# Rouslan/NTracer

Measured on AMD Instinct MI355X. Metric: Mrays/s (primary+shadow), 6-D hypercube @1920x1080, higher is better.
Workload: dtype f32

## Files before the change

ntracer_amd/csrc/nt_box.hpp:

```cpp
#pragma once
#include <type_traits>
#include "nt_pixel.hpp"

namespace {

__device__ __forceinline__ bool box_may_hit(int n, const float *dots, float sx, float sy, float sq) {
    const float osq = dots[0];
    const float ov = fmaf(-dots[2], sy, fmaf(dots[1], sx, dots[3]));
    const float rad2 = (float)n * (1.0f + NT_FUZZ) * (1.0f + NT_FUZZ) * 1.001f;
#ifdef NT_EXP_SKIP_SLABS
    return false;
#else
    return !((osq - rad2) * sq > ov * ov * 1.0001f);
#endif
}

__device__ __forceinline__ void box_background(float in, float &r, float &g, float &b) {
    if (in > 0.0f) { r = in; g = in; b = in; }
    else { r = 0.0f; g = -in; b = -in; }
}

template <int N>
__device__ __forceinline__ void box_color(const float (&o)[N], const float (&dir)[N], bool maybe, float &r, float &g, float &b) {
    bool done = false;
    float shade = 0.0f;

    {
        float num[N];
        bool pre[N];
        float aK = 0.0f, bK = 1.0f, oK = 0.0f;
        bool any = false;
#pragma unroll
        for (int i = 0; i < N; ++i) {
            const float di = dir[i];
            const float s = di < 0.0f ? 1.0f : -1.0f;
            num[i] = s - o[i];
            pre[i] = maybe && ((num[i] > 0.0f && di > 0.0f) || (num[i] < 0.0f && di < 0.0f));
            const float a = fabsf(num[i]), bb = fabsf(di);
            if (pre[i] && (!any || a * bK > aK * bb)) { aK = a; bK = bb; oK = o[i]; any = true; }
        }
        const float mu = 1e-4f * (1.0f + fabsf(oK));
        const float aKm = (aK - mu) * (1.0f - 1e-6f);
#pragma unroll
        for (int i = 0; i < N; ++i) {
            const bool tie = pre[i] && !done && !(fabsf(num[i]) * bK < fabsf(dir[i]) * aKm);
            if (__builtin_amdgcn_ballot_w64(tie) != 0ull) {
                const float di = dir[i];
                const float dist = num[i] / di;
                bool ok = tie && dist > 0.0f;
#pragma unroll
                for (int j = 0; j < N; ++j) {
                    if (j != i) {
                        const float p = dir[j] * dist + o[j];
                        ok = ok && !(fabsf(p) > (1.0f + NT_FUZZ));
                    }
                }
                if (ok) {
                    done = true;
                    if (dist >= FLT_MAX) shade = -1.0f;
                    else {
                        const float sine = di * (di < 0.0f ? 1.0f : -1.0f);
                        shade = sine <= 0.0f ? -sine : 0.0f;
                    }
                }
            }
        }
    }
    if (done && shade >= 0.0f) {
        r = shade * 1.0f;
        g = shade * 0.5f;
        b = shade * 0.5f;
    } else {
        box_background(dir[0], r, g, b);
    }
}

#ifndef NT_BOX_INLINE_MAX_N
#define NT_BOX_INLINE_MAX_N 8
#endif
#ifndef NT_BOX_SETS_MAX_N
#define NT_BOX_SETS_MAX_N NT_BOX_INLINE_MAX_N
#endif
#ifndef NT_BOX_MARGIN
#define NT_BOX_MARGIN 1e-5f
#endif
template <int N>
__device__ __forceinline__ void box_classify(const float (&o)[N], const float (&v)[N], float m, bool maybe, bool &hit, bool &unclear,
                                             float &x, float (&near)[N], float &tn, float &vK) {
    float tn2 = -INFINITY;
    tn = -INFINITY;
    vK = 0.0f;
    float tnp = -INFINITY, tfp = INFINITY;
    const float m1p = 1.0f + m;
#pragma unroll
    for (int j = 0; j < N; ++j) {
        const float inv = __builtin_amdgcn_rcpf(v[j]);
        const float c0 = -o[j] * inv;
        const float nr = c0 - fabsf(inv);
        near[j] = nr;
        tnp = fmaxf(tnp, fmaf(-fabsf(inv), m1p, c0));
        tfp = fminf(tfp, fmaf(fabsf(inv), m1p, c0));
        const bool later = nr > tn;
        tn2 = __builtin_amdgcn_fmed3f(tn, tn2, nr);
        vK = later ? v[j] : vK;
        tn = fmaxf(tn, nr);
    }
    const bool miss = tnp > tfp || tfp < 0.0f;
    const float c = 1.0f - m;
    float sum = 0.0f;
#pragma unroll
    for (int j = 0; j < N; ++j) sum = sum + fmaxf(fabsf(fmaf(v[j], tn, o[j])), c);
    const bool inside = sum - (float)N * c <= 1.5f * m;
    const bool sole = (tn - tn2) * fabsf(vK) > m;
    const bool front = tn > 1e-3f && tn < 1e30f;
    hit = maybe && !miss && inside && sole && front;
    unclear = maybe && !miss && !hit;
#ifdef NT_EXP_NOUNCLEAR
    unclear = false;
#endif
    x = hit ? vK : v[0];
}

__device__ __forceinline__ float nt_vmax(float a, float b) { float r; asm("v_max_f32 %0, %1, %2" : "=v"(r) : "v"(a), "v"(b)); return r; }
__device__ __forceinline__ float nt_vmin(float a, float b) { float r; asm("v_min_f32 %0, %1, %2" : "=v"(r) : "v"(a), "v"(b)); return r; }
__device__ __forceinline__ float nt_vmax3(float a, float b, float c) { float r; asm("v_max3_f32 %0, %1, %2, %3" : "=v"(r) : "v"(a), "v"(b), "v"(c)); return r; }
__device__ __forceinline__ float nt_vmin3(float a, float b, float c) { float r; asm("v_min3_f32 %0, %1, %2, %3" : "=v"(r) : "v"(a), "v"(b), "v"(c)); return r; }
__device__ __forceinline__ float nt_vmed3(float a, float b, float c) { float r; asm("v_med3_f32 %0, %1, %2, %3" : "=v"(r) : "v"(a), "v"(b), "v"(c)); return r; }
__device__ __forceinline__ float nt_vmax_abs(float a, float b) { float r; asm("v_max_f32 %0, |%1|, %2" : "=v"(r) : "v"(a), "v"(b)); return r; }

#ifndef NT_BOX_CLASSIFY_SETS_MIN_N
#define NT_BOX_CLASSIFY_SETS_MIN_N 6
#endif
#ifndef NT_BOX_CLASSIFY_SETS_MAX_N
#define NT_BOX_CLASSIFY_SETS_MAX_N 7
#endif
template <int N>
__device__ __forceinline__ void box_classify_sets(const float (&o)[N], const float (&v)[N], float m, uint32_t sets, bool &hit, bool &unclear,
                                                  float &x) {
    float tn = -INFINITY, tn2 = -INFINITY, vK = 0.0f;
    float tnp = -INFINITY, tfp = INFINITY;
    const float m1p = 1.0f + m;
#pragma unroll
    for (int j = 0; j < N; ++j) {
        if (((sets >> (10 + j)) & 1u) != 0u) {
            const float inv = __builtin_amdgcn_rcpf(v[j]);
            const float c0 = -o[j] * inv;
            tfp = nt_vmin(tfp, fmaf(fabsf(inv), m1p, c0));
            if (((sets >> j) & 1u) != 0u) {
                const float nr = c0 - fabsf(inv);
                tnp = nt_vmax(tnp, fmaf(-fabsf(inv), m1p, c0));
                const bool later = nr > tn;
                tn2 = nt_vmed3(tn, tn2, nr);
                vK = later ? v[j] : vK;
                tn = nt_vmax(tn, nr);
            }
        }
    }
    const bool miss = tnp > tfp || tfp < 0.0f;
    const float c = 1.0f - m;
    float sum = 0.0f;
#pragma unroll
    for (int j = 0; j < N; ++j) {
        if (((sets >> (10 + j)) & 1u) != 0u) {
            asm volatile("" : "+v"(sum));
            sum = sum + nt_vmax_abs(fmaf(v[j], tn, o[j]), c);
        }
    }
    const bool inside = sum - (float)__builtin_popcount((sets >> 10) & 0x3ffu) * c <= 1.5f * m;
    const bool sole = (tn - tn2) * fabsf(vK) > m;
    const bool front = tn > 1e-3f && tn < 1e30f;
    hit = !miss && inside && sole && front;
    unclear = !miss && !hit;
    x = hit ? vK : v[0];
}

template <int N>
__device__ __forceinline__ void box_entries(const float (&o)[N], const float (&v)[N], float (&near)[N], float &tn, float &vK) {
    tn = -INFINITY;
    vK = 0.0f;
#pragma unroll
    for (int j = 0; j < N; ++j) {
        const float inv = __builtin_amdgcn_rcpf(v[j]);
        const float nr = fmaf(-o[j], inv, -fabsf(inv));
        near[j] = nr;
        vK = nr > tn ? v[j] : vK;
        tn = fmaxf(tn, nr);
    }
}

template <int N>
__device__ __forceinline__ void box_resolve(const float (&o)[N], const float (&v)[N], float len, float m, const float (&near)[N], float tn,
                                            float vK, bool unclear, bool &hit, float &x) {
    const float aK = fabsf(vK);
    const float slack = m * __builtin_amdgcn_rcpf(aK), lim = 1.0f - 0.5f * m;
    bool inT[N], inC[N];
    float d[N];
    uint32_t anyC = 0u;
#pragma unroll
    for (int j = 0; j < N; ++j) {
        const bool early = (tn - near[j]) * aK > m;
        const bool robust = fmaf(fabsf(v[j]), slack, fabsf(fmaf(v[j], tn, o[j]))) <= lim;
        inT[j] = unclear && !early;
        inC[j] = unclear && !(robust && early);
        d[j] = 0.0f;
        if (__builtin_amdgcn_ballot_w64(inC[j]) != 0ull) {
            d[j] = v[j] / len;
            anyC |= 1u << j;
        }
    }
    bool done = false, found = false;
    float xs = v[0];
#pragma unroll
    for (int i = 0; i < N; ++i) {
        const bool cand = inT[i] && !done;
        if (__builtin_amdgcn_ballot_w64(cand) != 0ull) {
            const float di = d[i];
            const float dist = ((di < 0.0f ? 1.0f : -1.0f) - o[i]) / di;
            bool ok = cand && di != 0.0f && dist > 0.0f;
#pragma unroll
            for (int j = 0; j < N; ++j) {
                if (j != i && ((anyC >> j) & 1u) != 0u) {
                    const float p = d[j] * dist + o[j];
                    ok = ok && !(inC[j] && fabsf(p) > (1.0f + NT_FUZZ));
                }
            }
            if (ok) {
                done = true;
                if (!(dist >= FLT_MAX)) { found = true; xs = v[i]; }
            }
        }
    }
    if (unclear) {
        hit = found;
        x = xs;
    }
}

typedef __attribute__((address_space(1))) uint8_t *nt_gptr;
__device__ __forceinline__ nt_gptr uniform_ptr(uint8_t *p) {
    const unsigned long long v = reinterpret_cast<unsigned long long>(p);
    const uint32_t lo = (uint32_t)__builtin_amdgcn_readfirstlane((int)(uint32_t)v), hi = (uint32_t)__builtin_amdgcn_readfirstlane((int)(uint32_t)(v >> 32));
    return (nt_gptr)(((unsigned long long)hi << 32) | lo);
}
#define NT_G32(p) (*(__attribute__((address_space(1))) uint32_t *)(p))

template <typename P>
__device__ __forceinline__ void emit_f32x3_at(const NtTarget &tg, P p, float r, float gb) {
    r = r > 0.0f ? r : 0.0f;
    r = r < 1.0f ? r : 1.0f;
    gb = gb > 0.0f ? gb : 0.0f;
    gb = gb < 1.0f ? gb : 1.0f;
    uint32_t vr = __float_as_uint(r), vgb = __float_as_uint(gb);
    uint3 w;
    if (tg.plain_f32[0] == 0 && tg.plain_f32[1] == 1 && tg.plain_f32[2] == 2 && !tg.reversed) {
        w.x = bswap32(vr);
        w.y = bswap32(vgb);
        w.z = w.y;
    } else {
        if (!tg.reversed) { vr = bswap32(vr); vgb = bswap32(vgb); }
        w.x = tg.plain_f32[tg.reversed ? 2 : 0] == 0 ? vr : vgb;
        w.y = tg.plain_f32[1] == 0 ? vr : vgb;
        w.z = tg.plain_f32[tg.reversed ? 0 : 2] == 0 ? vr : vgb;
    }
    if constexpr (std::is_same<P, nt_gptr>::value) {
        typedef uint32_t u32x3 __attribute__((ext_vector_type(3)));
        u32x3 v;
        v.x = w.x; v.y = w.y; v.z = w.z;
        *(__attribute__((address_space(1))) u32x3 *)(p) = v;
    } else {
        *reinterpret_cast<uint3 *>(p) = w;
    }
}
__device__ __forceinline__ void emit_f32x3(const NtTarget &tg, long long offset, float r, float gb) { emit_f32x3_at(tg, tg.dest + offset, r, gb); }

__device__ __forceinline__ float sqrt_in_range(float x) {
    const float s = __builtin_amdgcn_sqrtf(x);
    const float s_dn = __uint_as_float(__float_as_uint(s) - 1u), s_up = __uint_as_float(__float_as_uint(s) + 1u);
    const float vp = fmaf(-s_dn, s, x), vs = fmaf(-s_up, s, x);
    float r = vp <= 0.0f ? s_dn : s;
    r = vs > 0.0f ? s_up : r;
    return r;
}
__device__ __forceinline__ float sqrt_wave(float x) {
    if (__builtin_amdgcn_ballot_w64(!(x >= 0x1p-96f && x < 0x1p96f)) == 0ull) return sqrt_in_range(x);
    return sqrtf(x);
}

template <int N, bool PLAIN, bool DEFER = false, bool REDO = false, bool F32 = false>
__device__ __forceinline__ bool box_pixel(const NtTarget &tg, const PixelRef &pr, const float (&org)[N], float (&dir)[N], float sq,
                                          const float (&dots)[4], float sx, float sy, float margin, bool rowhit = true, int face = -1,
                                          uint32_t sets = 0u, bool noclass = false) {
    constexpr bool INL = (F32 || PLAIN) && !REDO && !DEFER;
    const bool redo = REDO || (INL && noclass);
    const bool maybe = redo || (rowhit && (DEFER || INL || box_may_hit(N, dots, sx, sy, sq)));
    float r, g, b;
    bool hit = false, unclear = false;
    float x = dir[0];
#ifndef NT_EXP_NOCLASSIFY
    float near[N], tn = 0.0f, vK = 0.0f;
    constexpr bool CSETS = INL && N >= NT_BOX_CLASSIFY_SETS_MIN_N && N <= NT_BOX_CLASSIFY_SETS_MAX_N;
    auto exact_on_sets = [&]() {
        const float len = sqrt_wave(sq);
        float d[N];
#pragma unroll
        for (int j = 0; j < N; ++j) {
            d[j] = 0.0f;
            if ((sets >> (10 + j)) & 1u) d[j] = dir[j] / len;
        }
        bool done = false;
        x = dir[0];
#pragma unroll
        for (int i = 0; i < N; ++i) {
            if (((sets >> i) & 1u) != 0u && __builtin_amdgcn_ballot_w64(!done) != 0ull) {
// ... 245 lines not shown
    }
}

template <int N, bool SETS = false>
__device__ __forceinline__ unsigned long long box_stretch_code2(const float (&org)[N], const float (&right)[N], const float (&up)[N],
                                                                const float (&fwd)[N], const NtTarget &tg, int y, int col) {
    uint32_t sets_value = 0u;
    uint32_t *const sets = SETS ? &sets_value : nullptr;
    uint32_t code = 0u;
    float omax = fabsf(org[0]);
#pragma unroll
    for (int j = 1; j < N; ++j) omax = fmaxf(omax, fabsf(org[j]));
    const float m = NT_BOX_MARGIN * (1.0f + omax);
    const float h = 1.0f + 2.0f * m + 1e-3f;
    const float sxc = tg.fovI * (((float)(col * 64) + 31.5f) - tg.half_w);
    const float sy = tg.fovI * ((float)y - tg.half_h);
    const float spread = 32.0f * tg.fovI;
    float tlo = 0.0f, thi = INFINITY;
    float vc[N], g[N];
    float tn = -INFINITY, tn2 = -INFINITY, vK = 0.0f, gK = 0.0f, oK = 0.0f;
    int K = 0;
#pragma unroll
    for (int j = 0; j < N; ++j) {
        vc[j] = (fwd[j] + right[j] * sxc) - up[j] * sy;
        g[j] = fmaf(spread, fabsf(right[j]), 1e-6f);
        const float pa = vc[j] + g[j], qa = -h - org[j];
        const float pb = vc[j] - g[j], qb = h - org[j];
        const float ra = qa * __builtin_amdgcn_rcpf(pa), rb = qb * __builtin_amdgcn_rcpf(pb);
        const bool ap = pa >= 0.0f, bp = pb >= 0.0f;
        const float lo_a = ap ? ra : -INFINITY, hi_a = ap ? INFINITY : ra;
        const float hi_b = bp ? rb : INFINITY, lo_b = bp ? -INFINITY : rb;
        tlo = nt_vmax3(tlo, lo_a, lo_b);
        thi = nt_vmin3(thi, hi_a, hi_b);
    }
    if (!(tlo > thi)) {
        code = 15u;
#pragma unroll
        for (int j = 0; j < N; ++j) {
            const float nr = ((vc[j] < 0.0f ? 1.0f : -1.0f) - org[j]) * __builtin_amdgcn_rcpf(vc[j]);
            tn2 = nt_vmed3(tn, tn2, nr);
            const bool later = nr > tn;
            vK = later ? vc[j] : vK;
            gK = later ? g[j] : gK;
            oK = later ? org[j] : oK;
            K = later ? j : K;
            tn = nt_vmax(tn, nr);
        }
        const float vKa = vK - gK, vKb = vK + gK;
        if (K < 13 && vKa * vKb > 0.0f) {
            const float num = (vK < 0.0f ? 1.0f : -1.0f) - oK;
            const float t1 = num * __builtin_amdgcn_rcpf(vKa), t2 = num * __builtin_amdgcn_rcpf(vKb);
            const float t_lo = nt_vmin(t1, t2) * (1.0f - 1e-6f), t_hi = nt_vmax(t1, t2) * (1.0f + 1e-6f);
            const float rK = m * __builtin_amdgcn_rcpf(fabsf(vK) - gK) * (1.0f + 1e-6f);
            bool ok = t_lo > 1e-3f && t_hi < 1e30f;
#pragma unroll
            for (int j = 0; j < N; ++j) {
                const float va = vc[j] - g[j], vb = vc[j] + g[j];
                const float pmax = org[j] + nt_vmax(vb * t_lo, vb * t_hi);
                const float pmin = org[j] + nt_vmin(va * t_lo, va * t_hi);
                const float lim = (1.0f - m - 1e-4f) - (fabsf(vc[j]) + g[j]) * rK;
                ok = ok && (j == K || (pmax <= lim && pmin >= -lim));
            }
            if (ok) code = (uint32_t)K + 1u;
        }
        if (code == 15u && !((tn - tn2) * fabsf(vK) > m)) code = 14u;
        if (code >= 14u) {
            if (sets != nullptr && N <= 10) {
                auto range = [&](int j, float &A, float &B, float &vabs) {
                    const float va = vc[j] - g[j], vb = vc[j] + g[j];
                    const float num = (vc[j] < 0.0f ? 1.0f : -1.0f) - org[j];
                    const float e1 = num * __builtin_amdgcn_rcpf(va), e2 = num * __builtin_amdgcn_rcpf(vb);
                    const float lo = nt_vmin(e1, e2), hi = nt_vmax(e1, e2);
                    const bool same = va * vb > 0.0f;
                    A = same ? lo - fabsf(lo) * 1e-6f : -INFINITY;
                    B = same ? hi + fabsf(hi) * 1e-6f : INFINITY;
                    vabs = same ? fabsf(vc[j]) - g[j] : 0.0f;
                };
                float rA[N], rB[N], rV[N];
                float TN = -INFINITY, TH = -INFINITY;
#pragma unroll
                for (int j = 0; j < N; ++j) {
                    range(j, rA[j], rB[j], rV[j]);
                    TN = nt_vmax(TN, rA[j]);
                    TH = nt_vmax(TH, rB[j]);
                }
                float vmin = INFINITY;
#pragma unroll
                for (int j = 0; j < N; ++j) vmin = rB[j] >= TN ? nt_vmin(vmin, rV[j]) : vmin;
                const float M = m * __builtin_amdgcn_rcpf(vmin) * (1.0f + 1e-5f);
                uint32_t T = 0u, C = 0u;
                float t_lo = INFINITY;
                const float t_hi = TH;
#pragma unroll
                for (int j = 0; j < N; ++j) {
                    const bool inT = rB[j] >= TN - M;
                    T |= inT ? 1u << j : 0u;
                    t_lo = inT ? nt_vmin(t_lo, rA[j]) : t_lo;
                }
#pragma unroll
                for (int j = 0; j < N; ++j) {
                    const float va = vc[j] - g[j], vb = vc[j] + g[j];
                    const float pmax = org[j] + nt_vmax(vb * t_lo, vb * t_hi);
                    const float pmin = org[j] + nt_vmin(va * t_lo, va * t_hi);
                    const float lim = 1.0f - m - 1e-4f;
                    const bool inC = ((T >> j) & 1u) != 0u || !(pmax <= lim && pmin >= -lim);
                    C |= inC ? 1u << j : 0u;
                }
                const bool valid = vmin > 0.0f && t_lo > 1e-3f && t_hi < 1e30f;
                *sets = valid ? (0x80000000u | (C << 10) | T) : 0u;
            }
        }
    }
    return (unsigned long long)code | ((unsigned long long)sets_value << 32);
}
template <int N>
__device__ __forceinline__ uint32_t box_stretch_code(const float (&org)[N], const float (&right)[N], const float (&up)[N], const float (&fwd)[N],
                                                     const NtTarget &tg, int y, int col) {
    return (uint32_t)box_stretch_code2<N, false>(org, right, up, fwd, tg, y, col);
}

template <int N>
__global__ __launch_bounds__(256) void box_cull_kernel(NtCameraFixed cam, NtTarget tg, uint32_t *out, int ncols) {
    float org[N], right[N], up[N], fwd[N];
    load_camera<N>(cam, org, right, up, fwd);
    const int word = (int)blockIdx.x, row = (int)blockIdx.y * 8 + (int)(threadIdx.x >> 5);
    const int col = word * 32 + (int)(threadIdx.x & 31);
    uint32_t code = 0u;
    if (row < tg.row_count && col < ncols) {
        const int orow = tg.row_begin + row;
        int y = orow;
        if (tg.band_world > 1) {
            const int band = orow / tg.band_rows;
            y = (band * tg.band_world + tg.band_rank) * tg.band_rows + (orow - band * tg.band_rows);
        }
        code = box_stretch_code<N>(org, right, up, fwd, tg, y, col);
    }
    uint32_t packed = code << (4 * (threadIdx.x & 7));
    packed |= (uint32_t)__shfl_xor((int)packed, 1, 64);
    packed |= (uint32_t)__shfl_xor((int)packed, 2, 64);
    packed |= (uint32_t)__shfl_xor((int)packed, 4, 64);
    if (row < tg.row_count && (threadIdx.x & 7) == 0) out[((size_t)blockIdx.z * tg.row_count + row) * tg.cull_words + (col >> 3)] = packed;
}

#ifdef NT_EXP_NOSTORE
#define NT_EXP_STORE_IF if (tg.width < 0)
#else
#define NT_EXP_STORE_IF
#endif
#ifndef NT_TILE_OCC
#define NT_TILE_OCC
#endif
#ifndef NT_BOX_PIN_UP
#define NT_BOX_PIN_UP 1
#endif
template <int N, bool F32, int ROWS, int WAVES>
__global__ __launch_bounds__(64 * WAVES) NT_TILE_OCC void box_tile_kernel(NtCameraFixed cam, NtTarget tg) {
    static_assert(ROWS == 8 || ROWS == 16 || ROWS == 32 || ROWS == 64, "sixteen row codes to a qword, one to four qwords a wave");
    static_assert(WAVES >= 1 && WAVES <= 4 && WAVES * ROWS <= 64, "the codes of a tile are the work of one wave, a row per lane");
    constexpr int R = ROWS;
    __shared__ uint32_t s_code[64];
    __shared__ unsigned long long s_rows[4];
    constexpr bool ALLIN = F32 || N <= NT_BOX_INLINE_MAX_N;
    constexpr bool SETS_LDS = ALLIN && N <= NT_BOX_SETS_MAX_N;
    __shared__ uint32_t s_sets[SETS_LDS ? 64 : 1];
    __shared__ int s_abort;
    const int tid = (int)threadIdx.x;
    const int lane = tid & 63;
    const int wv = __builtin_amdgcn_readfirstlane(tid >> 6);
#ifdef NT_EXP_TRACE
    const unsigned long long trace_t0 = wall_clock64();
    unsigned trace_rows = 0u;
    unsigned long long trace_t1 = 0ull;
#endif
    const unsigned nframes = gridDim.z - (unsigned)tg.lead_frames;
    unsigned frame = blockIdx.z;
    if (tg.lead_frames > 0) {
        const unsigned cols = gridDim.x, q = cols / 4u;
        const bool middle = blockIdx.x >= q && blockIdx.x < cols - q;
        if (!middle) frame -= (unsigned)tg.lead_frames;
        if (frame >= nframes) return;
    }
    float org[N], right[N], up[N], fwd[N], dir[N];
    load_camera<N>(cam, frame, org, right, up, fwd);
    float margin = fabsf(org[0]);
#pragma unroll
    for (int j = 1; j < N; ++j) margin = fmaxf(margin, fabsf(org[j]));
    margin = NT_BOX_MARGIN * (1.0f + margin);
    float dots[4];
    if (cam.buf) {
        const float *dp = cam.dots + (size_t)frame * 4;
        dots[0] = dp[0]; dots[1] = dp[1]; dots[2] = dp[2]; dots[3] = dp[3];
    } else {
        dots[0] = cam.odots[0]; dots[1] = cam.odots[1]; dots[2] = cam.odots[2]; dots[3] = cam.odots[3];
    }
    const int tile_row0 = (int)blockIdx.y * WAVES * R;
    if (wv == (int)((blockIdx.x + blockIdx.y + frame) % (unsigned)WAVES)) {
        if (tg.abort_word != nullptr) {
            const bool ab = nt_aborted(tg);
            if (WAVES == 1) { if (ab) return; }
            else if (lane == 0) s_abort = ab ? 1 : 0;
        }
        uint32_t code = 0u;
        uint32_t row_sets = 0u;
        const int trow = tg.row_il > 0 ? ((int)blockIdx.y * WAVES + lane / R) + tg.row_il * (lane % R) : tile_row0 + lane;
        if (lane < WAVES * R && trow < tg.row_count) {
            const int orow = tg.row_begin + trow;
            int y = orow;
            if (tg.band_world > 1) {
                const int band = orow / tg.band_rows;
                y = (band * tg.band_world + tg.band_rank) * tg.band_rows + (orow - band * tg.band_rows);
            }
            if (y < tg.height) {
                const unsigned long long cs = box_stretch_code2<N, (N <= NT_BOX_SETS_MAX_N)>(org, right, up, fwd, tg, y, (int)blockIdx.x);
                code = (uint32_t)cs;
                row_sets = (uint32_t)(cs >> 32);
            }
        }
        if (SETS_LDS) s_sets[lane] = row_sets;
        {
            const unsigned long long m0 = __builtin_amdgcn_ballot_w64(code == 0u), m1 = __builtin_amdgcn_ballot_w64(code >= 1u && code <= 13u),
                                     m2 = __builtin_amdgcn_ballot_w64(code == 15u), m3 = __builtin_amdgcn_ballot_w64(code == 14u);
            if (lane == 0) {
                s_rows[0] = m0;
                s_rows[1] = m1;
                s_rows[2] = m2;
                s_rows[3] = m3;
            }
        }
        uint32_t packed = code << (4 * (lane & 7));
        packed |= (uint32_t)__shfl_xor((int)packed, 1, 64);
        packed |= (uint32_t)__shfl_xor((int)packed, 2, 64);
        packed |= (uint32_t)__shfl_xor((int)packed, 4, 64);
        if ((lane & 7) == 0) {
            const int grp = lane >> 3;
            const int slot = R == 8 ? 2 * grp : grp;
            s_code[slot] = packed;
            if (R == 8) s_code[slot + 1] = 0u;
        }
    }
    __syncthreads();
    if (WAVES > 1 && tg.abort_word != nullptr && s_abort != 0) return;
#ifdef NT_EXP_TRACE
    trace_t1 = wall_clock64();
#endif
    constexpr int HALVES = R >= 32 ? R / 16 : 1, RH = R / HALVES;
    const int wrow0 = tile_row0 + wv * R;
    const int il = tg.row_il;
    const int wfirst = il > 0 ? (int)blockIdx.y * WAVES + wv : wrow0;
    if (wfirst < tg.row_count) {
        typedef uint32_t nt_u32x4 __attribute__((ext_vector_type(4)));
        typedef __attribute__((address_space(4))) const nt_u32x4 *nt_rowtab;
        uint8_t *const frame_base = tg.dest + (long long)frame * tg.frame_stride;
#define NT_ROW_LOAD(rr)                     \
        const nt_u32x4 row_e = tab[(rr)];   \
        const float sy = __uint_as_float(row_e.x)
#define NT_ROW_OFF() ((long long)(((unsigned long long)row_e.w << 32) | row_e.z) + (long long)frame * tg.frame_stride)
#define NT_ROW_PTR() uniform_ptr(frame_base + (long long)(((unsigned long long)row_e.w << 32) | row_e.z))
#define NT_LANE_OFF() ({ asm volatile("" : "+v"(xoff)); xoff; })
#define NT_CLEAR_BIT(mask, bit) asm("s_bitset0_b32 %0, %1" : "+s"(mask) : "s"(bit))
        int x = (int)blockIdx.x * 64 + lane;
        x = x < tg.width ? x : tg.width - 1;
        uint32_t xoff = (uint32_t)x * (uint32_t)tg.bpp;
        const float sx = tg.fovI * ((float)x - tg.half_w);
        float base[N];
#pragma unroll
        for (int j = 0; j < N; ++j) base[j] = fwd[j] + right[j] * sx;
        float upv[N];
#pragma unroll
        for (int j = 0; j < N; ++j) {
            upv[j] = up[j];
            if (NT_BOX_PIN_UP || F32 || j == 0) asm volatile("" : "+v"(upv[j]));
        }
        float bb = 0.0f, bu = 0.0f, uu = 0.0f;
        bool fastsq = true;
        if (!F32) {
#pragma unroll
            for (int j = 0; j < N; ++j) {
                bb = fmaf(base[j], base[j], bb);
                bu = fmaf(base[j], up[j], bu);
                uu = fmaf(up[j], up[j], uu);
            }
            fastsq = __builtin_amdgcn_ballot_w64(!(bu * bu <= bb * uu * 0.0625f)) == 0ull;
        }
        const float maxv = (float)tg.plain_maxval;
        const float inv_maxv2 = 1.0f / (maxv * maxv);
        const float m2bu = (-2.0f * bu) * inv_maxv2;
        bb = bb * inv_maxv2;
        uu = uu * inv_maxv2;
        auto rows_of = [&](int k) {
            const unsigned long long m = s_rows[k];
            return (((unsigned long long)(uint32_t)__builtin_amdgcn_readfirstlane((int)(uint32_t)(m >> 32)) << 32) |
                    (uint32_t)__builtin_amdgcn_readfirstlane((int)(uint32_t)m)) >> (wv * R);
        };
        const unsigned long long rows_culled = rows_of(0), rows_face = rows_of(1), rows_rays = rows_of(2), rows_tie = rows_of(3);
#pragma unroll 1
        for (int half = 0; half < HALVES; ++half) {
        const int row0 = wrow0 + 16 * half;
        const int hfirst = il > 0 ? wfirst + il * 16 * half : row0;
        if (hfirst >= tg.row_count) break;
        uint32_t redo_bits = 0u;
        const int cw = (R >= 32 ? (R / 8) * wv + 2 * half : 2 * wv);
        unsigned long long rowcodes = ((unsigned long long)(uint32_t)__builtin_amdgcn_readfirstlane((int)s_code[cw + 1]) << 32) |
                                      (uint32_t)__builtin_amdgcn_readfirstlane((int)s_code[cw]);
        const int lrow = il > 0 ? hfirst + il * lane : row0 + lane;
        const int lorow = tg.row_begin + lrow;
        int ly = lorow;
        if (tg.band_world > 1) {
            const int band = lorow / tg.band_rows;
            ly = (band * tg.band_world + tg.band_rank) * tg.band_rows + (lorow - band * tg.band_rows);
        }
        const uint32_t valid = (uint32_t)__builtin_amdgcn_ballot_w64(lane < RH && lrow < tg.row_count && ly < tg.height);
        const nt_rowtab tab = (nt_rowtab)tg.rowtab + (il > 0 ? row0 : tg.row_begin + row0);
        uint32_t quick = (uint32_t)(rows_culled >> (16 * half)) & valid, inner = (uint32_t)(rows_face >> (16 * half)) & valid;
        uint32_t todo = (uint32_t)((ALLIN ? rows_rays | rows_tie : rows_rays) >> (16 * half)) & valid;
        if (!ALLIN) redo_bits = (uint32_t)(rows_tie >> (16 * half)) & valid;
#ifdef NT_EXP_TRACE
        trace_rows += (unsigned)__builtin_popcount(quick) | ((unsigned)__builtin_popcount(inner) << 8) |
                      ((unsigned)__builtin_popcount((uint32_t)(rows_rays >> (16 * half)) & valid) << 16) |
                      ((unsigned)__builtin_popcount((uint32_t)(rows_tie >> (16 * half)) & valid) << 24);
#endif
        if (!F32) {
            if (!fastsq) {
                todo |= quick | inner;
                quick = 0u;
                inner = 0u;
            }
            auto lean_rows = [&](auto sel8) {
            constexpr bool SEL8 = decltype(sel8)::value;
            while (quick != 0u) {
                const int rr = __builtin_ctz(quick);
                NT_CLEAR_BIT(quick, rr);
                NT_ROW_LOAD(rr);
                const float d0 = base[0] - upv[0] * sy;
                const float sqa = fmaf(sy, fmaf(sy, uu, m2bu), bb);
                const float t = fabsf(d0) * __builtin_amdgcn_rsqf(sqa);
                const bool clear = fabsf(__builtin_amdgcn_fractf(t) - 0.5f) > fmaf(t, 0x1p-18f, 0x1p-18f);
                if (__builtin_amdgcn_ballot_w64(!clear) != 0ull) {
                    todo |= 1u << rr;
                    continue;
                }
                const nt_gptr out = NT_ROW_PTR() + NT_LANE_OFF();
                if (SEL8) {
                    const uint32_t q = __float_as_uint(t + 8388608.0f);
                    const uint32_t w = __builtin_amdgcn_perm(d0 > 0.0f ? q : 0u, q, tg.plain_sel);
                    NT_EXP_STORE_IF NT_G32(out) = w;
                    continue;
                }
                uint32_t q = (uint32_t)(t + 0.5f);
                q = q < tg.plain_maxval ? q : tg.plain_maxval;
                const uint32_t w = (d0 > 0.0f ? q : 0u) * tg.plain_mul[0] + q * (tg.plain_mul[1] + tg.plain_mul[2]);
                NT_EXP_STORE_IF NT_G32(out) = tg.reversed ? w : bswap32(w);
            }
            uint32_t K0 = 0u;
            float bK0 = base[0], uK0 = upv[0];
            if (inner != 0u) {
                K0 = ((uint32_t)(rowcodes >> (4 * __builtin_ctz(inner))) & 15u) - 1u;
#pragma unroll
                for (int j = 1; j < N; ++j) {
                    bK0 = K0 == (uint32_t)j ? base[j] : bK0;
                    uK0 = K0 == (uint32_t)j ? upv[j] : uK0;
                }
            }
            while (inner != 0u) {
                const int rr = __builtin_ctz(inner);
                NT_CLEAR_BIT(inner, rr);
                const uint32_t K = ((uint32_t)(rowcodes >> (4 * rr)) & 15u) - 1u;
                NT_ROW_LOAD(rr);
                float bK = bK0, uK = uK0;
                if (K != K0) {
                    bK = base[0];
                    uK = upv[0];
#pragma unroll
                    for (int j = 1; j < N; ++j) {
                        bK = K == (uint32_t)j ? base[j] : bK;
                        uK = K == (uint32_t)j ? upv[j] : uK;
                    }
                }
                const float dK = bK - uK * sy;
                const float sqa = fmaf(sy, fmaf(sy, uu, m2bu), bb);
                const float t = fabsf(dK) * __builtin_amdgcn_rsqf(sqa), th = t * 0.5f;
                const bool clear = fabsf(__builtin_amdgcn_fractf(t) - 0.5f) > fmaf(t, 0x1p-18f, 0x1p-18f) &&
                                   fabsf(__builtin_amdgcn_fractf(th) - 0.5f) > fmaf(th, 0x1p-18f, 0x1p-18f);
                if (__builtin_amdgcn_ballot_w64(!clear) != 0ull) {
                    todo |= 1u << rr;
                    continue;
                }
                const nt_gptr out = NT_ROW_PTR() + NT_LANE_OFF();
                if (SEL8) {
                    NT_EXP_STORE_IF NT_G32(out) = __builtin_amdgcn_perm(__float_as_uint(t + 8388608.0f), __float_as_uint(th + 8388608.0f), tg.plain_sel);
                    continue;
                }
                uint32_t qr = (uint32_t)(t + 0.5f), qgb = (uint32_t)(th + 0.5f);
                qr = qr < tg.plain_maxval ? qr : tg.plain_maxval;
                qgb = qgb < tg.plain_maxval ? qgb : tg.plain_maxval;
                const uint32_t w = qr * tg.plain_mul[0] + qgb * (tg.plain_mul[1] + tg.plain_mul[2]);
                NT_EXP_STORE_IF NT_G32(out) = tg.reversed ? w : bswap32(w);
            }
            };
            if (tg.plain_sel != 0u) lean_rows(std::true_type{});
            else lean_rows(std::false_type{});
        } else {
            while (quick != 0u) {
                const int rr = __builtin_ctz(quick);
                quick &= quick - 1u;
                NT_ROW_LOAD(rr);
#pragma unroll
                for (int j = 0; j < N; ++j) dir[j] = base[j] - upv[j] * sy;
                float sq = dir[0] * dir[0];
#pragma unroll
                for (int j = 1; j < N; ++j) sq = sq + dir[j] * dir[j];
                const float in = dir[0] / sqrt_wave(sq);
                float r, gb, b_;
                box_background(in, r, gb, b_);
                emit_f32x3_at(tg, NT_ROW_PTR() + NT_LANE_OFF(), r, gb);
            }
            uint32_t K0 = 0u;
            float bK0 = base[0], uK0 = upv[0];
            if (inner != 0u) {
                K0 = ((uint32_t)(rowcodes >> (4 * __builtin_ctz(inner))) & 15u) - 1u;
#pragma unroll
                for (int j = 1; j < N; ++j) {
                    bK0 = K0 == (uint32_t)j ? base[j] : bK0;
                    uK0 = K0 == (uint32_t)j ? upv[j] : uK0;
                }
            }
            while (inner != 0u) {
                const int rr = __builtin_ctz(inner);
                inner &= inner - 1u;
                const uint32_t K = ((uint32_t)(rowcodes >> (4 * rr)) & 15u) - 1u;
                NT_ROW_LOAD(rr);
#pragma unroll
                for (int j = 0; j < N; ++j) dir[j] = base[j] - upv[j] * sy;
                float sq = dir[0] * dir[0];
#pragma unroll
                for (int j = 1; j < N; ++j) sq = sq + dir[j] * dir[j];
                float bK = bK0, uK = uK0;
                if (K != K0) {
                    bK = base[0];
                    uK = upv[0];
#pragma unroll
                    for (int j = 1; j < N; ++j) {
                        bK = K == (uint32_t)j ? base[j] : bK;
                        uK = K == (uint32_t)j ? upv[j] : uK;
                    }
                }
                const float xk = bK - uK * sy;
                const float shade = fabsf(xk / sqrt_wave(sq));
                emit_f32x3_at(tg, NT_ROW_PTR() + NT_LANE_OFF(), shade * 1.0f, shade * 0.5f);
            }
        }
        while (todo != 0u) {
            const int rr = __builtin_ctz(todo);
            todo &= todo - 1u;
            const bool rowhit = ((uint32_t)(rowcodes >> (4 * rr)) & 15u) != 0u;
            NT_ROW_LOAD(rr);
            PixelRef pr;
            pr.x = x;
            pr.y = 0;
            pr.offset = NT_ROW_OFF() + (long long)xoff;
            pr.hit_index = 0;
            pr.valid = true;
#pragma unroll
            for (int j = 0; j < N; ++j) dir[j] = base[j] - upv[j] * sy;
            float sq = dir[0] * dir[0];
#pragma unroll
            for (int j = 1; j < N; ++j) sq = sq + dir[j] * dir[j];
            const int rcode = (int)((uint32_t)(rowcodes >> (4 * rr)) & 15u);
            if (ALLIN) {
                uint32_t sets = 0u;
                if (SETS_LDS) sets = (uint32_t)__builtin_amdgcn_readfirstlane((int)s_sets[wv * R + 16 * half + rr]);
                box_pixel<N, !F32, false, false, F32>(tg, pr, org, dir, sq, dots, sx, sy, margin, rowhit, rcode >= 1 && rcode <= 13 ? rcode - 1 : -1, sets,
                                                       rcode == 14);
            } else if (!box_pixel<N, true, true, false, false>(tg, pr, org, dir, sq, dots, sx, sy, margin, rowhit, rcode >= 1 && rcode <= 13 ? rcode - 1 : -1)) {
                redo_bits |= 1u << rr;
            }
        }
        if (!ALLIN && lane == 0) {
            while (redo_bits != 0u) {
                const int rr = __builtin_ctz(redo_bits);
                redo_bits &= redo_bits - 1u;
                const int mrow = il > 0 ? hfirst + il * rr : row0 + rr;
                atomicOr(tg.redo + ((size_t)frame * tg.row_count + mrow) * tg.redo_words + (blockIdx.x >> 5), 1u << (blockIdx.x & 31));
            }
        }
        }
    }
#ifdef NT_EXP_TRACE
    if (lane == 0) {
        unsigned long long *tr = reinterpret_cast<unsigned long long *>(tg.dest + (long long)nframes * tg.frame_stride) +
                                 ((((size_t)frame * gridDim.y + blockIdx.y) * gridDim.x + blockIdx.x) * WAVES + wv) * 4;
        tr[0] = trace_t0;
        tr[1] = wall_clock64();
        tr[2] = (unsigned long long)__builtin_amdgcn_s_getreg(4 | (31 << 11)) | ((unsigned long long)__builtin_amdgcn_s_getreg(20 | (31 << 11)) << 32);
        tr[3] = (unsigned long long)trace_rows | ((trace_t1 - trace_t0) << 32);
    }
#endif
#undef NT_ROW_LOAD
#undef NT_ROW_OFF
#undef NT_ROW_PTR
#undef NT_LANE_OFF
#undef NT_CLEAR_BIT
}

template <int N>
int launch_box_fixed(const NtLaunchInfo &li, const NtCamera &cam, const NtTarget &tg_in) {
    NtCameraFixed cf;
    cf.buf = cam.buf;
    cf.dots = cam.dots;
    for (int k = 0; k < 4; ++k) cf.odots[k] = cam.odots[k];
    cf.n = N;
    for (int k = 0; k < 4 * N; ++k) cf.inl[k] = cam.inl[k];
    NtTarget tg = tg_in;
    dim3 grid;
    grid_for(tg, 64, tg.colors_out ? 4 : 4 * NT_BOXROWS, li.nframes, grid);
    tg.cull = nullptr;
    tg.redo = nullptr;
    tg.cull_words = 0;
    tg.redo_words = 0;
    const bool fmt_rgb = tg.plain_bits != 0u && tg.plain_bits <= 10u && tg.bpp == 4 && tg.aligned4;
    const bool fmt_f32 = tg.plain_f32[0] >= 0 && tg.bpp == 12 && tg.aligned4;
    if (li.cull_buf && tg.rowtab && !tg.colors_out && (fmt_rgb || fmt_f32) && li.cull_clean) {
        hipStream_t st = (hipStream_t)li.stream;
        NtBoxTileGeom geom;
        geom.rows = li.tile_rows;
        geom.waves = li.tile_waves;
        const bool r64 = geom.rows == 64, r16 = geom.rows == 16;
        const int wpb = geom.waves;
        const int tile_rows = geom.rows * geom.waves;
        dim3 tgrid((unsigned)((tg.width + 63) / 64), (unsigned)((tg.row_count + tile_rows - 1) / tile_rows), (unsigned)li.nframes);
        tg.redo_words = ((tg.width + 63) / 64 + 31) / 32;
        tg.redo = li.cull_buf;
        tg.lead_frames = li.nframes >= 8 ? (li.nframes < 96 ? li.nframes : 96) : 0;
        if (tg.row_il > 0) tg.lead_frames = li.nframes >= 32 ? 16 : 0;
        if ((long long)li.nframes + tg.lead_frames > 65535) tg.lead_frames = 0;
        tgrid.z += (unsigned)tg.lead_frames;
        if (fmt_rgb) {
            if (r64) hipLaunchKernelGGL((box_tile_kernel<N, false, 64, 1>), tgrid, dim3(64), 0, st, cf, tg);
            else if (r16 && wpb == 3) hipLaunchKernelGGL((box_tile_kernel<N, false, 16, 3>), tgrid, dim3(192), 0, st, cf, tg);
            else if (r16) hipLaunchKernelGGL((box_tile_kernel<N, false, 16, 4>), tgrid, dim3(256), 0, st, cf, tg);
            else hipLaunchKernelGGL((box_tile_kernel<N, false, 8, 4>), tgrid, dim3(256), 0, st, cf, tg);
            if constexpr (N > NT_BOX_INLINE_MAX_N) {
                const long long rwords = (long long)tg.row_count * li.nframes * tg.redo_words;
                const int split = rwords < 48 * 1024 ? 2 : 1;
                const int rpb = 4 / split;
                const dim3 rgrid((unsigned)tg.redo_words, (unsigned)((tg.row_count + rpb - 1) / rpb), (unsigned)li.nframes);
                if (split == 2) hipLaunchKernelGGL((box_redo_kernel<N, 2>), rgrid, dim3(256), 0, st, cf, tg);
                else hipLaunchKernelGGL((box_redo_kernel<N, 1>), rgrid, dim3(256), 0, st, cf, tg);
            }
        } else {
            if (r64) hipLaunchKernelGGL((box_tile_kernel<N, true, 64, 1>), tgrid, dim3(64), 0, st, cf, tg);
            else if (r16 && wpb == 3) hipLaunchKernelGGL((box_tile_kernel<N, true, 16, 3>), tgrid, dim3(192), 0, st, cf, tg);
            else if (r16) hipLaunchKernelGGL((box_tile_kernel<N, true, 16, 4>), tgrid, dim3(256), 0, st, cf, tg);
            else hipLaunchKernelGGL((box_tile_kernel<N, true, 8, 4>), tgrid, dim3(256), 0, st, cf, tg);
        }
        return 0;
    }
    if (li.cull_buf && !tg.colors_out) {
        const int ncols = (tg.width + 63) / 64;
        const int words = (ncols + 31) / 32;
        tg.cull_words = 4 * words;
        hipLaunchKernelGGL(box_cull_kernel<N>, dim3((unsigned)words, (unsigned)((tg.row_count + 7) / 8), (unsigned)li.nframes), dim3(256), 0,
                           (hipStream_t)li.stream, cf, tg, li.cull_buf, ncols);
        tg.cull = li.cull_buf;
    }
    hipLaunchKernelGGL(box_kernel<N>, grid, dim3(256), 0, (hipStream_t)li.stream, cf, tg);
    return 0;
}

}
```

Before: 1.001 million.

## Process lean rows in aligned groups of four with one wide row-table load

For mid-range dimensions, quick (culled) and single-face rows are now handled in aligned groups of four. Each group reads its four row-table entries with one 64-byte scalar load, evaluates all four, and issues the four stores together. Leftover rows, and face groups whose axis differs from the first one, fall back to the per-row loop. Row validity is also ballot-computed once per wave instead of once per half, and the `sets` mask is pinned to a scalar register. The aim is to cut scalar-load latency and per-row loop overhead, at the cost of more code, higher register pressure and extra branching.

```diff
diff --git a/ntracer_amd/csrc/nt_box.hpp b/ntracer_amd/csrc/nt_box.hpp
--- a/ntracer_amd/csrc/nt_box.hpp
+++ b/ntracer_amd/csrc/nt_box.hpp
@@ -159,6 +159,9 @@
     const bool miss = tnp > tfp || tfp < 0.0f;
     const float c = 1.0f - m;
     float sum = 0.0f;
+#ifndef NT_EXP_SETS_MASKS
+    asm volatile("" : "+s"(sets));
+#endif
 #pragma unroll
     for (int j = 0; j < N; ++j) {
         if (((sets >> (10 + j)) & 1u) != 0u) {
@@ -710,6 +713,12 @@
 #endif
 #ifndef NT_BOX_PIN_UP
 #define NT_BOX_PIN_UP 1
+#endif
+#ifndef NT_BOX_LEAN_GROUPS_MIN_N
+#define NT_BOX_LEAN_GROUPS_MIN_N 3
+#endif
+#ifndef NT_BOX_LEAN_GROUPS_MAX_N
+#define NT_BOX_LEAN_GROUPS_MAX_N 20
 #endif
 template <int N, bool F32, int ROWS, int WAVES>
 __global__ __launch_bounds__(64 * WAVES) NT_TILE_OCC void box_tile_kernel(NtCameraFixed cam, NtTarget tg) {
@@ -808,14 +817,20 @@
     if (wfirst < tg.row_count) {
         typedef uint32_t nt_u32x4 __attribute__((ext_vector_type(4)));
         typedef __attribute__((address_space(4))) const nt_u32x4 *nt_rowtab;
+        typedef uint32_t nt_u32x16 __attribute__((ext_vector_type(16), aligned(16)));
+        typedef __attribute__((address_space(4))) const nt_u32x16 *nt_rowtab4;
+        constexpr bool LEAN4 = N >= NT_BOX_LEAN_GROUPS_MIN_N && N <= NT_BOX_LEAN_GROUPS_MAX_N;
+        constexpr bool GROUPS = !F32 && LEAN4;
         uint8_t *const frame_base = tg.dest + (long long)frame * tg.frame_stride;
 #define NT_ROW_LOAD(rr)                     \
         const nt_u32x4 row_e = tab[(rr)];   \
         const float sy = __uint_as_float(row_e.x)
 #define NT_ROW_OFF() ((long long)(((unsigned long long)row_e.w << 32) | row_e.z) + (long long)frame * tg.frame_stride)
 #define NT_ROW_PTR() uniform_ptr(frame_base + (long long)(((unsigned long long)row_e.w << 32) | row_e.z))
+#define NT_GROUP_PTR(k) uniform_ptr(frame_base + (long long)(((unsigned long long)grp_e[4 * (k) + 3] << 32) | grp_e[4 * (k) + 2]))
 #define NT_LANE_OFF() ({ asm volatile("" : "+v"(xoff)); xoff; })
 #define NT_CLEAR_BIT(mask, bit) asm("s_bitset0_b32 %0, %1" : "+s"(mask) : "s"(bit))
+#define NT_SET_BIT(mask, bit) asm("s_bitset1_b32 %0, %1" : "+s"(mask) : "s"(bit))
         int x = (int)blockIdx.x * 64 + lane;
         x = x < tg.width ? x : tg.width - 1;
         uint32_t xoff = (uint32_t)x * (uint32_t)tg.bpp;
@@ -851,6 +866,17 @@
                     (uint32_t)__builtin_amdgcn_readfirstlane((int)(uint32_t)m)) >> (wv * R);
         };
         const unsigned long long rows_culled = rows_of(0), rows_face = rows_of(1), rows_rays = rows_of(2), rows_tie = rows_of(3);
+        unsigned long long rows_valid = 0ull;
+        if (LEAN4) {
+            const int lrow = il > 0 ? wfirst + il * lane : wrow0 + lane;
+            const int lorow = tg.row_begin + lrow;
+            int ly = lorow;
+            if (tg.band_world > 1) {
+                const int band = lorow / tg.band_rows;
+                ly = (band * tg.band_world + tg.band_rank) * tg.band_rows + (lorow - band * tg.band_rows);
+            }
+            rows_valid = __builtin_amdgcn_ballot_w64(lane < R && lrow < tg.row_count && ly < tg.height);
+        }
 #pragma unroll 1
         for (int half = 0; half < HALVES; ++half) {
         const int row0 = wrow0 + 16 * half;
@@ -860,14 +886,19 @@
         const int cw = (R >= 32 ? (R / 8) * wv + 2 * half : 2 * wv);
         unsigned long long rowcodes = ((unsigned long long)(uint32_t)__builtin_amdgcn_readfirstlane((int)s_code[cw + 1]) << 32) |
                                       (uint32_t)__builtin_amdgcn_readfirstlane((int)s_code[cw]);
-        const int lrow = il > 0 ? hfirst + il * lane : row0 + lane;
-        const int lorow = tg.row_begin + lrow;
-        int ly = lorow;
-        if (tg.band_world > 1) {
-            const int band = lorow / tg.band_rows;
-            ly = (band * tg.band_world + tg.band_rank) * tg.band_rows + (lorow - band * tg.band_rows);
-        }
-        const uint32_t valid = (uint32_t)__builtin_amdgcn_ballot_w64(lane < RH && lrow < tg.row_count && ly < tg.height);
+        uint32_t valid;
+        if (LEAN4) {
+            valid = HALVES > 1 ? (uint32_t)(rows_valid >> (16 * half)) & 0xffffu : (uint32_t)rows_valid;
+        } else {
+            const int lrow = il > 0 ? hfirst + il * lane : row0 + lane;
+            const int lorow = tg.row_begin + lrow;
+            int ly = lorow;
+            if (tg.band_world > 1) {
+                const int band = lorow / tg.band_rows;
+                ly = (band * tg.band_world + tg.band_rank) * tg.band_rows + (lorow - band * tg.band_rows);
+            }
+            valid = (uint32_t)__builtin_amdgcn_ballot_w64(lane < RH && lrow < tg.row_count && ly < tg.height);
+        }
         const nt_rowtab tab = (nt_rowtab)tg.rowtab + (il > 0 ? row0 : tg.row_begin + row0);
         uint32_t quick = (uint32_t)(rows_culled >> (16 * half)) & valid, inner = (uint32_t)(rows_face >> (16 * half)) & valid;
         uint32_t todo = (uint32_t)((ALLIN ? rows_rays | rows_tie : rows_rays) >> (16 * half)) & valid;
@@ -885,74 +916,219 @@
             }
             auto lean_rows = [&](auto sel8) {
             constexpr bool SEL8 = decltype(sel8)::value;
-            while (quick != 0u) {
-                const int rr = __builtin_ctz(quick);
-                NT_CLEAR_BIT(quick, rr);
-                NT_ROW_LOAD(rr);
-                const float d0 = base[0] - upv[0] * sy;
-                const float sqa = fmaf(sy, fmaf(sy, uu, m2bu), bb);
-                const float t = fabsf(d0) * __builtin_amdgcn_rsqf(sqa);
-                const bool clear = fabsf(__builtin_amdgcn_fractf(t) - 0.5f) > fmaf(t, 0x1p-18f, 0x1p-18f);
-                if (__builtin_amdgcn_ballot_w64(!clear) != 0ull) {
-                    todo |= 1u << rr;
-                    continue;
-                }
-                const nt_gptr out = NT_ROW_PTR() + NT_LANE_OFF();
+            auto put_quick = [&](nt_gptr out, float t, float d0) {
                 if (SEL8) {
                     const uint32_t q = __float_as_uint(t + 8388608.0f);
-                    const uint32_t w = __builtin_amdgcn_perm(d0 > 0.0f ? q : 0u, q, tg.plain_sel);
-                    NT_EXP_STORE_IF NT_G32(out) = w;
-                    continue;
+                    NT_EXP_STORE_IF NT_G32(out) = __builtin_amdgcn_perm(d0 > 0.0f ? q : 0u, q, tg.plain_sel);
+                    return;
                 }
                 uint32_t q = (uint32_t)(t + 0.5f);
                 q = q < tg.plain_maxval ? q : tg.plain_maxval;
                 const uint32_t w = (d0 > 0.0f ? q : 0u) * tg.plain_mul[0] + q * (tg.plain_mul[1] + tg.plain_mul[2]);
                 NT_EXP_STORE_IF NT_G32(out) = tg.reversed ? w : bswap32(w);
-            }
-            uint32_t K0 = 0u;
-            float bK0 = base[0], uK0 = upv[0];
-            if (inner != 0u) {
-                K0 = ((uint32_t)(rowcodes >> (4 * __builtin_ctz(inner))) & 15u) - 1u;
-#pragma unroll
-                for (int j = 1; j < N; ++j) {
-                    bK0 = K0 == (uint32_t)j ? base[j] : bK0;
-                    uK0 = K0 == (uint32_t)j ? upv[j] : uK0;
-                }
-            }
-            while (inner != 0u) {
-                const int rr = __builtin_ctz(inner);
-                NT_CLEAR_BIT(inner, rr);
-                const uint32_t K = ((uint32_t)(rowcodes >> (4 * rr)) & 15u) - 1u;
-                NT_ROW_LOAD(rr);
-                float bK = bK0, uK = uK0;
-                if (K != K0) {
-                    bK = base[0];
-                    uK = upv[0];
-#pragma unroll
-                    for (int j = 1; j < N; ++j) {
-                        bK = K == (uint32_t)j ? base[j] : bK;
-                        uK = K == (uint32_t)j ? upv[j] : uK;
-                    }
-                }
-                const float dK = bK - uK * sy;
-                const float sqa = fmaf(sy, fmaf(sy, uu, m2bu), bb);
-                const float t = fabsf(dK) * __builtin_amdgcn_rsqf(sqa), th = t * 0.5f;
-                const bool clear = fabsf(__builtin_amdgcn_fractf(t) - 0.5f) > fmaf(t, 0x1p-18f, 0x1p-18f) &&
-                                   fabsf(__builtin_amdgcn_fractf(th) - 0.5f) > fmaf(th, 0x1p-18f, 0x1p-18f);
-                if (__builtin_amdgcn_ballot_w64(!clear) != 0ull) {
-                    todo |= 1u << rr;
-                    continue;
-                }
-                const nt_gptr out = NT_ROW_PTR() + NT_LANE_OFF();
+            };
+            auto put_face = [&](nt_gptr out, float t, float th) {
                 if (SEL8) {
                     NT_EXP_STORE_IF NT_G32(out) = __builtin_amdgcn_perm(__float_as_uint(t + 8388608.0f), __float_as_uint(th + 8388608.0f), tg.plain_sel);
-                    continue;
+                    return;
                 }
                 uint32_t qr = (uint32_t)(t + 0.5f), qgb = (uint32_t)(th + 0.5f);
                 qr = qr < tg.plain_maxval ? qr : tg.plain_maxval;
                 qgb = qgb < tg.plain_maxval ? qgb : tg.plain_maxval;
                 const uint32_t w = qr * tg.plain_mul[0] + qgb * (tg.plain_mul[1] + tg.plain_mul[2]);
                 NT_EXP_STORE_IF NT_G32(out) = tg.reversed ? w : bswap32(w);
+            };
+            auto full_groups = [](uint32_t mask) { return mask & (mask >> 1) & (mask >> 2) & (mask >> 3) & 0x1111u; };
+            if (GROUPS) {
+                uint32_t full = full_groups(quick);
+                quick &= ~(full * 15u);
+                while (full != 0u) {
+                    const int g = __builtin_ctz(full);
+                    NT_CLEAR_BIT(full, g);
+                    const nt_u32x16 grp_e = *(nt_rowtab4)(tab + g);
+                    float t[4], d0[4];
+                    unsigned long long fail[4];
+#pragma unroll
+                    for (int k = 0; k < 4; ++k) {
+                        const float sy = __uint_as_float(grp_e[4 * k]);
+                        d0[k] = base[0] - upv[0] * sy;
+                        const float sqa = fmaf(sy, fmaf(sy, uu, m2bu), bb);
+                        t[k] = fabsf(d0[k]) * __builtin_amdgcn_rsqf(sqa);
+                        const bool clear = fabsf(__builtin_amdgcn_fractf(t[k]) - 0.5f) > fmaf(t[k], 0x1p-18f, 0x1p-18f);
+                        fail[k] = __builtin_amdgcn_ballot_w64(!clear);
+                    }
+                    if (__builtin_expect(((fail[0] | fail[1]) | (fail[2] | fail[3])) == 0ull, 1)) {
+                        const uint32_t xo = NT_LANE_OFF();
+                        put_quick(NT_GROUP_PTR(0) + xo, t[0], d0[0]);
+                        put_quick(NT_GROUP_PTR(1) + xo, t[1], d0[1]);
+                        put_quick(NT_GROUP_PTR(2) + xo, t[2], d0[2]);
+                        put_quick(NT_GROUP_PTR(3) + xo, t[3], d0[3]);
+                    } else {
+                        todo |= ((fail[0] != 0ull ? 1u : 0u) | (fail[1] != 0ull ? 2u : 0u) | (fail[2] != 0ull ? 4u : 0u) | (fail[3] != 0ull ? 8u : 0u)) << g;
+#pragma unroll
+                        for (int k = 0; k < 4; ++k) {
+                            if (fail[k] == 0ull) {
+                                uint32_t xo = xoff;
+                                asm volatile("" : "+v"(xo));
+                                put_quick(NT_GROUP_PTR(k) + xo, t[k], d0[k]);
+                            }
+                        }
+                    }
+                }
+                uint32_t quick_stored = 0u;
+                for (uint32_t rest = quick; rest != 0u;) {
+                    const int rr = __builtin_ctz(rest);
+                    NT_CLEAR_BIT(rest, rr);
+                    NT_ROW_LOAD(rr);
+                    const float d0 = base[0] - upv[0] * sy;
+                    const float sqa = fmaf(sy, fmaf(sy, uu, m2bu), bb);
+                    const float t = fabsf(d0) * __builtin_amdgcn_rsqf(sqa);
+                    const bool clear = fabsf(__builtin_amdgcn_fractf(t) - 0.5f) > fmaf(t, 0x1p-18f, 0x1p-18f);
+                    if (__builtin_expect(__builtin_amdgcn_ballot_w64(!clear) == 0ull, 1)) {
+                        put_quick(NT_ROW_PTR() + NT_LANE_OFF(), t, d0);
+                        NT_SET_BIT(quick_stored, rr);
+                    }
+                }
+                todo |= quick & ~quick_stored;
+            } else {
+                while (quick != 0u) {
+                    const int rr = __builtin_ctz(quick);
+                    NT_CLEAR_BIT(quick, rr);
+                    NT_ROW_LOAD(rr);
+                    const float d0 = base[0] - upv[0] * sy;
+                    const float sqa = fmaf(sy, fmaf(sy, uu, m2bu), bb);
+                    const float t = fabsf(d0) * __builtin_amdgcn_rsqf(sqa);
+                    const bool clear = fabsf(__builtin_amdgcn_fractf(t) - 0.5f) > fmaf(t, 0x1p-18f, 0x1p-18f);
+                    if (__builtin_amdgcn_ballot_w64(!clear) != 0ull) {
+                        todo |= 1u << rr;
+                        continue;
+                    }
+                    const nt_gptr out = NT_ROW_PTR() + NT_LANE_OFF();
+                    if (SEL8) {
+                        const uint32_t q = __float_as_uint(t + 8388608.0f);
+                        const uint32_t w = __builtin_amdgcn_perm(d0 > 0.0f ? q : 0u, q, tg.plain_sel);
+                        NT_EXP_STORE_IF NT_G32(out) = w;
+                        continue;
+                    }
+                    uint32_t q = (uint32_t)(t + 0.5f);
+                    q = q < tg.plain_maxval ? q : tg.plain_maxval;
+                    const uint32_t w = (d0 > 0.0f ? q : 0u) * tg.plain_mul[0] + q * (tg.plain_mul[1] + tg.plain_mul[2]);
+                    NT_EXP_STORE_IF NT_G32(out) = tg.reversed ? w : bswap32(w);
+                }
+            }
+            uint32_t K0 = 0u;
+            float bK0 = base[0], uK0 = upv[0];
+            if (inner != 0u) {
+                K0 = ((uint32_t)(rowcodes >> (4 * __builtin_ctz(inner))) & 15u) - 1u;
+#pragma unroll
+                for (int j = 1; j < N; ++j) {
+                    bK0 = K0 == (uint32_t)j ? base[j] : bK0;
+                    uK0 = K0 == (uint32_t)j ? upv[j] : uK0;
+                }
+            }
+            if (GROUPS) {
+                uint32_t full = full_groups(inner);
+                const uint32_t same = (K0 + 1u) * 0x1111u;
+                while (full != 0u) {
+                    const int g = __builtin_ctz(full);
+                    NT_CLEAR_BIT(full, g);
+                    if (((uint32_t)(rowcodes >> (4 * g)) & 0xffffu) != same) continue;
+                    const nt_u32x16 grp_e = *(nt_rowtab4)(tab + g);
+                    inner &= ~(15u << g);
+                    float t[4], th[4];
+                    unsigned long long fail[4];
+#pragma unroll
+                    for (int k = 0; k < 4; ++k) {
+                        const float sy = __uint_as_float(grp_e[4 * k]);
+                        const float dK = bK0 - uK0 * sy;
+                        const float sqa = fmaf(sy, fmaf(sy, uu, m2bu), bb);
+                        t[k] = fabsf(dK) * __builtin_amdgcn_rsqf(sqa);
+                        th[k] = t[k] * 0.5f;
+                        const bool clear = fabsf(__builtin_amdgcn_fractf(t[k]) - 0.5f) > fmaf(t[k], 0x1p-18f, 0x1p-18f) &&
+                                           fabsf(__builtin_amdgcn_fractf(th[k]) - 0.5f) > fmaf(th[k], 0x1p-18f, 0x1p-18f);
+                        fail[k] = __builtin_amdgcn_ballot_w64(!clear);
+                    }
+                    if (__builtin_expect(((fail[0] | fail[1]) | (fail[2] | fail[3])) == 0ull, 1)) {
+                        const uint32_t xo = NT_LANE_OFF();
+                        put_face(NT_GROUP_PTR(0) + xo, t[0], th[0]);
+                        put_face(NT_GROUP_PTR(1) + xo, t[1], th[1]);
+                        put_face(NT_GROUP_PTR(2) + xo, t[2], th[2]);
+                        put_face(NT_GROUP_PTR(3) + xo, t[3], th[3]);
+                    } else {
+                        todo |= ((fail[0] != 0ull ? 1u : 0u) | (fail[1] != 0ull ? 2u : 0u) | (fail[2] != 0ull ? 4u : 0u) | (fail[3] != 0ull ? 8u : 0u)) << g;
+#pragma unroll
+                        for (int k = 0; k < 4; ++k) {
+                            if (fail[k] == 0ull) {
+                                uint32_t xo = xoff;
+                                asm volatile("" : "+v"(xo));
+                                put_face(NT_GROUP_PTR(k) + xo, t[k], th[k]);
+                            }
+                        }
+                    }
+                }
+                uint32_t inner_stored = 0u;
+                for (uint32_t rest = inner; rest != 0u;) {
+                    const int rr = __builtin_ctz(rest);
+                    NT_CLEAR_BIT(rest, rr);
+                    const uint32_t K = ((uint32_t)(rowcodes >> (4 * rr)) & 15u) - 1u;
+                    NT_ROW_LOAD(rr);
+                    float bK = bK0, uK = uK0;
+                    if (K != K0) {
+                        bK = base[0];
+                        uK = upv[0];
+    #pragma unroll
+                        for (int j = 1; j < N; ++j) {
+                            bK = K == (uint32_t)j ? base[j] : bK;
+                            uK = K == (uint32_t)j ? upv[j] : uK;
+                        }
+                    }
+                    const float dK = bK - uK * sy;
+                    const float sqa = fmaf(sy, fmaf(sy, uu, m2bu), bb);
+                    const float t = fabsf(dK) * __builtin_amdgcn_rsqf(sqa), th = t * 0.5f;
+                    const bool clear = fabsf(__builtin_amdgcn_fractf(t) - 0.5f) > fmaf(t, 0x1p-18f, 0x1p-18f) &&
+                                       fabsf(__builtin_amdgcn_fractf(th) - 0.5f) > fmaf(th, 0x1p-18f, 0x1p-18f);
+                    if (__builtin_expect(__builtin_amdgcn_ballot_w64(!clear) == 0ull, 1)) {
+                        put_face(NT_ROW_PTR() + NT_LANE_OFF(), t, th);
+                        NT_SET_BIT(inner_stored, rr);
+                    }
+                }
+                todo |= inner & ~inner_stored;
+            } else {
+                while (inner != 0u) {
+                    const int rr = __builtin_ctz(inner);
+                    NT_CLEAR_BIT(inner, rr);
+                    const uint32_t K = ((uint32_t)(rowcodes >> (4 * rr)) & 15u) - 1u;
+                    NT_ROW_LOAD(rr);
+                    float bK = bK0, uK = uK0;
+                    if (K != K0) {
+                        bK = base[0];
+                        uK = upv[0];
+    #pragma unroll
+                        for (int j = 1; j < N; ++j) {
+                            bK = K == (uint32_t)j ? base[j] : bK;
+                            uK = K == (uint32_t)j ? upv[j] : uK;
+                        }
+                    }
+                    const float dK = bK - uK * sy;
+                    const float sqa = fmaf(sy, fmaf(sy, uu, m2bu), bb);
+                    const float t = fabsf(dK) * __builtin_amdgcn_rsqf(sqa), th = t * 0.5f;
+                    const bool clear = fabsf(__builtin_amdgcn_fractf(t) - 0.5f) > fmaf(t, 0x1p-18f, 0x1p-18f) &&
+                                       fabsf(__builtin_amdgcn_fractf(th) - 0.5f) > fmaf(th, 0x1p-18f, 0x1p-18f);
+                    if (__builtin_amdgcn_ballot_w64(!clear) != 0ull) {
+                        todo |= 1u << rr;
+                        continue;
+                    }
+                    const nt_gptr out = NT_ROW_PTR() + NT_LANE_OFF();
+                    if (SEL8) {
+                        NT_EXP_STORE_IF NT_G32(out) = __builtin_amdgcn_perm(__float_as_uint(t + 8388608.0f), __float_as_uint(th + 8388608.0f), tg.plain_sel);
+                        continue;
+                    }
+                    uint32_t qr = (uint32_t)(t + 0.5f), qgb = (uint32_t)(th + 0.5f);
+                    qr = qr < tg.plain_maxval ? qr : tg.plain_maxval;
+                    qgb = qgb < tg.plain_maxval ? qgb : tg.plain_maxval;
+                    const uint32_t w = qr * tg.plain_mul[0] + qgb * (tg.plain_mul[1] + tg.plain_mul[2]);
+                    NT_EXP_STORE_IF NT_G32(out) = tg.reversed ? w : bswap32(w);
+                }
             }
             };
             if (tg.plain_sel != 0u) lean_rows(std::true_type{});
@@ -1056,8 +1232,10 @@
 #undef NT_ROW_LOAD
 #undef NT_ROW_OFF
 #undef NT_ROW_PTR
+#undef NT_GROUP_PTR
 #undef NT_LANE_OFF
 #undef NT_CLEAR_BIT
+#undef NT_SET_BIT
 }
 
 template <int N>
```

After: 1.022 million, median of 6. 1.02x the previous value.
